# Daniel-Starr/pointcloudhookup

Measured on AMD Instinct MI355X. Metric: Mpts/s ground-filter+tower-cluster, 100 M-pt corridor; % HBM roofline on kNN, higher is better.
Workload: dtype f32 (filter) + f64 (distance predicate)

## Files before the change

### pointcloudhookup_amd/csrc/pch_filter.hip

```cpp
#include "pch_prims.h"
#include "pch_mean.h"
#include "pch_lookback.h"

namespace pch {

constexpr int SEL_BINS = 4096;
constexpr int SEL_REP0 = 4;
constexpr int SEL_TILE = 4096;

struct SelState {
    unsigned long long rank;
    unsigned long long less;
    uint32_t prefix;
    uint32_t need_next;
    uint32_t v0key;
    uint32_t pad;
};

__device__ __forceinline__ uint32_t sel_key(float v) {
    return (v != v) ? 0xFFFFFFFFu : f32_ordered(v);
}

template <int ROUNDS>
__device__ __forceinline__ void sel_hist_add(uint32_t* h, bool active, uint32_t bin) {
    bool pending = active;
#pragma unroll
    for (int round = 0; round < ROUNDS; ++round) {
        const unsigned long long todo = __ballot(pending);
        if (__popcll(todo) < 8) break;
        const int leader = (int)__builtin_ctzll(todo);
        const uint32_t b0 = (uint32_t)__builtin_amdgcn_readlane((int)bin, leader);
        const unsigned long long same = __ballot(pending && bin == b0);
        if (lane_id() == leader) atomicAdd(&h[b0], (uint32_t)__popcll(same));
        pending = pending && bin != b0;
    }
    if (pending) atomicAdd(&h[bin], 1u);
}

struct SelGate { const uint32_t* ok; const float* alt_base; const uint32_t* alt_n; };
__device__ __forceinline__ void sel_gate(const SelGate& g, const float*& base, int64_t& n, int64_t& stride) {
    if (g.ok && *g.ok) { base = g.alt_base; n = (int64_t)*g.alt_n; stride = 1; }
}

__device__ __forceinline__ float sel_key_to_float(uint32_t k) {
// ... 267 lines not shown
            float4 q[4];
#pragma unroll
            for (int r = 0; r < 4; ++r) q[r] = b4[r * 256 + threadIdx.x];
#pragma unroll
            for (int r = 0; r < 4; ++r) { take(true, q[r].x); take(true, q[r].y); take(true, q[r].z); take(true, q[r].w); }
        } else {
            for (int r = 0; r < SEL_TILE / 256; ++r) {
                const int64_t i = t0 + r * 256 + threadIdx.x;
                const bool in = i < n;
                take(in, in ? base[i] : 0.0f);
            }
        }
    }
    __syncthreads();
    flush();
    less = wave_reduce_add(less);
    nans = wave_reduce_add(nans);
    if (lane_id() == 0) {
        if (less) atomicAdd(&br->less, less);
        if (nans) atomicAdd(&br->nan, nans);
    }
}

__global__ void sel_bracket_fix_k(BrState* __restrict__ br, SelRun* __restrict__ run, unsigned long long k0, int same) {
    if (threadIdx.x != 0 || blockIdx.x != 0) return;
    const unsigned long long less = br->less, cnt = br->count;
    const bool ok = br->overflow == 0 && less <= k0 && (k0 - less) < cnt && (same || (k0 + 1 - less) < cnt);
    br->ok = ok ? 1u : 0u;
    SelState z;
    z.rank = ok ? k0 - less : k0;
    z.less = 0; z.prefix = 0; z.need_next = 0; z.v0key = 0; z.pad = 0;
    run->st[0] = z;
    run->nan_count = ok ? br->nan : 0ull;
}

__global__ __launch_bounds__(256) void sel_init_k(uint32_t* __restrict__ hist, int nwords, SelRun* __restrict__ runs,
                                                   int nruns, unsigned long long r0, unsigned long long r1,
                                                   unsigned long long r2, BrState* __restrict__ br,
                                                   uint32_t* __restrict__ also_zero, int64_t also_words) {
    const int i = blockIdx.x * 256 + threadIdx.x;
    if (i < nwords) hist[i] = 0;
    for (int64_t j = i; j < also_words; j += (int64_t)gridDim.x * 256) also_zero[j] = 0u;
    if (i < nruns) {
        SelRun z;
        memset(&z, 0, sizeof(z));
        z.st[0].rank = i == 0 ? r0 : (i == 1 ? r1 : r2);
        z.next_min = 0xFFFFFFFFu;
        runs[i] = z;
    }
    if (i == 0 && br) { BrState b; memset(&b, 0, sizeof(b)); *br = b; }
}

struct SelWs {
    float*    scal;
    SelRun*   run;
    uint32_t* hist;
    BrState*  br;
    float    *sample, *cand;
    int64_t   ns;
    uint32_t  cap;
    uint32_t* also_zero;
    int64_t   also_words;
};
static void sel_plan(Arena& a, SelWs& w, int64_t n = 0) {
    w.scal = a.take<float>(4);
    w.run = a.take<SelRun>(3);
    w.hist = a.take<uint32_t>(9 * SEL_BINS);
    w.br = nullptr; w.sample = w.cand = nullptr; w.ns = 0; w.cap = 0;
    w.also_zero = nullptr; w.also_words = 0;
    if (n >= SEL_BRACKET_MIN) {
        w.br = a.take<BrState>(1);
        w.ns = SEL_GROUP * (n / SEL_EVERY);
        w.sample = a.take<float>(w.ns);
        w.cap = (uint32_t)(n / 16) + 1024u;
        w.cand = a.take<float>(w.cap);
    }
}

struct PctIndex { int64_t k0; int same; float gamma; };
static PctIndex pct_index(int64_t n, double q_percent) {
    PctIndex r;
    const float q = (float)q_percent / 100.0f;
    const float vi = (float)(n - 1) * q;
    float prev = floorf(vi);
    r.gamma = vi - prev;
    r.same = 0;
    if (vi >= (float)(n - 1)) { prev = (float)(n - 1); r.same = 1; }
    if (vi < 0.0f) { prev = 0.0f; r.same = 1; }
    int64_t k0 = (int64_t)prev;
    if (k0 > n - 1) k0 = n - 1;
    if (k0 < 0) k0 = 0;
    if (k0 == n - 1) r.same = 1;
    r.k0 = k0;
    return r;
}

static int select_rounds(const float* base, int64_t n, int64_t stride, bool with_next, SelRun* run, uint32_t* hist,
                         hipStream_t s, SelGate gate, int64_t grid_n) {
    int64_t gb = ceil_div(grid_n, SEL_TILE);
    if (gb > 2048) gb = 2048;
    if (gb < 1) gb = 1;
    const dim3 grid((unsigned)gb), blk(256);
    PCH_LAUNCH("sel_hist0", (sel_hist_k<0, 1>), grid, blk, 0, s, base, n, stride, run, hist, gate);
    PCH_LAUNCH("sel_hist1", (sel_hist_k<1, 1>), grid, blk, 0, s, base, n, stride, run, hist, gate);
    PCH_LAUNCH("sel_hist2", (sel_hist_k<2, 1>), grid, blk, 0, s, base, n, stride, run, hist, gate);
    if (with_next) PCH_LAUNCH("sel_next", sel_next_k<>, grid, blk, 0, s, base, n, stride, run, hist, gate);
    return PCH_OK;
}

static bool select_is_bracketed(const SelWs& w, int64_t n, int64_t stride) {
    return w.sample && stride == 1 && n >= SEL_BRACKET_MIN;
}
struct SelBracket { int64_t r_lo, r_hi; };
static SelBracket select_bracket_ranks(const SelWs& w, int64_t n, const PctIndex& pi) {
    const int64_t ns = w.ns;
    const double p = (double)pi.k0 / (double)(n > 1 ? n - 1 : 1);
    const double sigma = sqrt(p * (1.0 - p) * (double)ns * 16.0);
    const int64_t margin = (int64_t)(6.0 * sigma) + ns / 500 + 16;
    const int64_t mid = (int64_t)(p * (double)(ns - 1));
    SelBracket r;
    r.r_lo = mid - margin < 0 ? 0 : mid - margin;
    r.r_hi = mid + margin > ns - 1 ? ns - 1 : mid + margin;
    return r;
}
static int select_sample_passes(const float* src, int64_t src_stride, int64_t n, double q_percent, SelWs& w,
                                hipStream_t s) {
    const PctIndex pi = pct_index(n, q_percent);
    const SelGate always = {nullptr, nullptr, nullptr};
    const SelBracket br = select_bracket_ranks(w, n, pi);
    const int64_t ns = w.ns;
    PCH_LAUNCH("sel_init", sel_init_k, dim3((unsigned)ceil_div(9 * SEL_BINS, 256)), dim3(256), 0, s, w.hist,
               9 * SEL_BINS, w.run, 3, (unsigned long long)br.r_lo, (unsigned long long)br.r_hi, 0ull, w.br,
               w.also_zero, w.also_words);
    PCH_LAUNCH("sel_sample", sel_sample_k, dim3((unsigned)ceil_div(ns, 1024)), dim3(256), 0, s, src, src_stride, ns,
               w.sample);
    int64_t gs = ceil_div(ns, SEL_TILE);
    if (gs > 2048) gs = 2048;
    if (gs < 1) gs = 1;
    const dim3 grid((unsigned)gs), blk(256);
    PCH_LAUNCH("sel_hist0", (sel_hist_k<0, 2>), grid, blk, 0, s, (const float*)w.sample, ns, (int64_t)1, w.run, w.hist, always);
    PCH_LAUNCH("sel_hist1", (sel_hist_k<1, 2>), grid, blk, 0, s, (const float*)w.sample, ns, (int64_t)1, w.run, w.hist, always);
    PCH_LAUNCH("sel_hist2", (sel_hist_k<2, 2>), grid, blk, 0, s, (const float*)w.sample, ns, (int64_t)1, w.run, w.hist, always);
    return PCH_OK;
}

static int select_passes(const float* base, int64_t n, int64_t stride, double q_percent, SelWs& w,
// ... 8 lines not shown
                   w.also_words);
        return select_rounds(base, n, stride, !pi.same, fin, hfin, s, always, n);
    }
    if (!sample_done) PCH_TRY(select_sample_passes(base, 1, n, q_percent, w, s));
    const SelBracket br = select_bracket_ranks(w, n, pi);
    const int64_t ns = w.ns;
    int64_t gb = ceil_div(n, SEL_TILE);
    {
        static int per_round[PCH_MAX_DEVICES] = {};
        const int slot = current_device_slot();
        if (!per_round[slot]) {
            int dev = 0, cus = 256;
            if (hipGetDevice(&dev) == hipSuccess) (void)hipDeviceGetAttribute(&cus, hipDeviceAttributeMultiprocessorCount, dev);
            per_round[slot] = cus * 5;
        }
        if (gb > per_round[slot]) gb = per_round[slot];
    }
    PCH_LAUNCH("sel_bracket", sel_bracket_k, dim3((unsigned)gb), dim3(256), 0, s, base, n, (const SelRun*)w.run, w.hist,
               br.r_lo == 0 ? 1 : 0, br.r_hi == ns - 1 ? 1 : 0, w.br, w.cand, w.cap);
    PCH_LAUNCH("sel_bracket_fix", sel_bracket_fix_k, dim3(1), dim3(64), 0, s, w.br, fin, (unsigned long long)pi.k0,
               pi.same);
    const SelGate src = {&w.br->ok, w.cand, &w.br->count};
    return select_rounds(base, n, stride, !pi.same, fin, hfin, s, src, n);
}
static int select_lerp(int64_t n, const float* sub, double q_percent, float add1, float add2, SelWs& w,
                       hipStream_t s) {
    const PctIndex pi = pct_index(n, q_percent);
    PCH_LAUNCH("sel_lerp", sel_lerp_k, dim3(1), dim3(256), 0, s, (const SelRun*)(w.run + 2),
               (const uint32_t*)(w.hist + 8 * SEL_BINS), pi.same ? 0 : 1, pi.same, pi.gamma, sub, add1, add2, w.scal);
    return PCH_OK;
}
static int select_percentile(const float* base, int64_t n, int64_t stride, const float* sub,
                             double q_percent, SelWs& w, hipStream_t s) {
    PCH_TRY(select_passes(base, n, stride, q_percent, w, s));
    return select_lerp(n, sub, q_percent, 0.0f, 0.0f, w, s);
}

struct SideStream { hipStream_t s; hipEvent_t ev_fork, ev_join, ev_start; bool ok; };
struct SideStreams {
    SideStream ss[PCH_MAX_DEVICES];
    SideStreams() { for (auto& x : ss) x = {nullptr, nullptr, nullptr, nullptr, false}; }
    ~SideStreams() {
        if (!may_release_hip_objects()) return;
        for (auto& x : ss)
            if (x.ok) {
                (void)hipEventDestroy(x.ev_fork); (void)hipEventDestroy(x.ev_join);
// ... 315 lines not shown
        out_scalars[5] = use_b ? 1.0f : 0.0f;
        out_scalars[6] = __uint_as_float(st->total[0]);
        out_scalars[7] = 0.0f;
        *out_count = st->failed ? (int64_t)-1 : (int64_t)st->total[use_b];
    }
    if (threadIdx.x < 6 && out_aabb) {
        const int a = threadIdx.x;
        uint32_t v = 0;
        for (int k = 0; k < GF_SLOTS; ++k) { const uint32_t u = st->slots[use_b][k][a]; v = u > v ? u : v; }
        out_aabb[a] = v == 0u ? 0.0f : f32_unordered(a < 3 ? ~v : v);
    }
}

struct GfWs {
    float*    centroid;
    float*    zcol;
    MsWs      ms;
    SelWs     sel;
    GfState*  st;
    uint64_t* status;
    size_t    clear_bytes;
    MsCand    cand;
};
static void gf_plan(Arena& a, int64_t n, GfWs& w) {
    const int64_t nb = ceil_div(n > 0 ? n : 1, GF_TILE);
    w.centroid = a.take<float>(4);
    ms_plan(a, n, w.ms);
    w.zcol = a.take<float>(n > 0 ? n : 1);
    sel_plan(a, w.sel, n);
    const size_t st_off = a.off;
    w.st = a.take<GfState>(1);
    w.status = a.take<uint64_t>(2 * nb);
    w.clear_bytes = a.off - st_off;
    const int64_t nblk = ceil_div(n > 0 ? n : 1, GF_CBLK);
    w.cand.tcand = a.take<float>(4);
    w.cand.counts = a.take<uint32_t>(nblk);
    w.cand.zsample = a.take<float>(nblk);
    w.cand.slots = a.take<float>(nblk * 4 * MS_CAND_SLOT);
    w.cand.pct = 0.0;
    w.cand.add = 0.0f;
}

}

using namespace pch;

extern "C" size_t pch_percentile_f32_ws_bytes(int64_t n) {
    Arena a;
    SelWs w;
    sel_plan(a, w, n);
    return a.off;
}

extern "C" int pch_percentile_f32(const float* base, int64_t n, int64_t stride, const float* sub,
                                  double q_percent, float* out, void* ws, size_t ws_bytes,
                                  void* stream) {
    PCH_DEVICE_GUARD(base);
    hipStream_t s = (hipStream_t)stream;
    PCH_REQUIRE(n >= 1, "percentile of an empty array (numpy raises IndexError)");
    PCH_REQUIRE(base && out && ws && stride >= 1, "bad argument");
    PCH_REQUIRE(q_percent >= 0.0 && q_percent <= 100.0, "Percentiles must be in the range [0, 100]");
    Arena a(ws, ws_bytes);
    SelWs w;
// ... 125 lines not shown
    return pch::ground_filter_run(raw, n, pct, offset, fallback_offset, min_keep, out_points, out_index, out_scalars,
                                  out_count, out_aabb, ws, ws_bytes, (hipStream_t)stream, nullptr);
}

int pch::ground_filter_run(const float* raw, int64_t n, double pct, float offset, float fallback_offset,
                           int64_t min_keep, float* out_points, int32_t* out_index, float* out_scalars,
                           int64_t* out_count, float* out_aabb, void* ws, size_t ws_bytes, hipStream_t s,
                           const GfEarly* early) {
    PCH_REQUIRE(n >= 1 && n < (int64_t(1) << 31), "n out of range [1, 2^31) (numpy raises on empty input)");
    PCH_REQUIRE(raw && out_points && out_scalars && out_count && ws, "null buffer");
    PCH_REQUIRE(pct >= 0.0 && pct <= 100.0, "Percentiles must be in the range [0, 100]");
    Arena a(ws, ws_bytes);
    GfWs w;
    gf_plan(a, n, w);
    if (a.overflow) { set_error("workspace too small: need %zu bytes", a.off); return PCH_ERR_WORKSPACE; }
    const int64_t nb = ceil_div(n, GF_TILE);

    w.cand.pct = pct;
    w.cand.add = (offset < fallback_offset ? offset : fallback_offset) - 0.5f;
    bool cand_made = false;
    w.sel.also_zero = reinterpret_cast<uint32_t*>(w.st);
    w.sel.also_words = (int64_t)(w.clear_bytes / 4);
    SideStream& ss = side_stream();
    const bool sample_early = ss.ok && select_is_bracketed(w.sel, n, 1);
    if (sample_early) {
        PCH_HIP_TRY(hipEventRecord(ss.ev_start, s));
        PCH_HIP_TRY(hipStreamWaitEvent(ss.s, ss.ev_start, 0));
        PCH_TRY(select_sample_passes(raw + 2, 3, n, pct, w.sel, ss.s));
    }
    PCH_TRY(mean_seq_launch(raw, n, w.centroid, w.ms, w.zcol, s, ss.ok ? ss.ev_fork : nullptr, nullptr, MS_DIVIDE_BY_N,
                            MS_PHASE_BOTH, &w.cand, &cand_made));
    if (ss.ok) PCH_HIP_TRY(hipStreamWaitEvent(ss.s, ss.ev_fork, 0));
    PCH_TRY(select_passes(w.zcol, n, 1, pct, w.sel, ss.ok ? ss.s : s, sample_early));
    if (ss.ok) {
        PCH_HIP_TRY(hipEventRecord(ss.ev_join, ss.s));
        PCH_HIP_TRY(hipStreamWaitEvent(s, ss.ev_join, 0));
    }
    PCH_TRY(select_lerp(n, w.centroid + 2, pct, offset, fallback_offset, w.sel, s));
    const dim3 grid((unsigned)nb), blk(GF_THREADS);
    const float* tcand = cand_made ? (const float*)w.cand.tcand : (const float*)nullptr;
    const int64_t nblk = ceil_div(n, GF_CBLK);
    const dim3 cgrid((unsigned)ceil_div(nblk, GF_CT_BLKS));
    if (cand_made)
        PCH_LAUNCH("gf_cand", gf_cand_k<0>, cgrid, blk, 0, s, (const float*)w.cand.slots, (const uint32_t*)w.cand.counts,
                   tcand, nblk, (const float*)w.centroid, (const float*)w.sel.scal, w.st, w.status, (long long)min_keep,
                   out_points, out_index);
    PCH_LAUNCH("gf_compact", gf_compact_k<0>, grid, blk, 0, s, raw, (const float*)w.zcol, n,
               (const float*)w.centroid, (const float*)w.sel.scal, w.st, w.status, (long long)min_keep, out_points,
               out_index, tcand);
    if (early) {
        PCH_LAUNCH("gf_finalize", gf_finalize_k, dim3(1), dim3(64), 0, s, (const GfState*)w.st,
                   (const float*)w.centroid, (const float*)w.sel.scal, out_scalars, out_count, out_aabb);
        PCH_TRY(peek_enqueue(early->dev, early->bytes, s));
    }
    if (cand_made)
        PCH_LAUNCH("gf_cand_fb", gf_cand_k<1>, cgrid, blk, 0, s, (const float*)w.cand.slots,
                   (const uint32_t*)w.cand.counts, tcand, nblk, (const float*)w.centroid, (const float*)w.sel.scal, w.st,
                   w.status + nb, (long long)min_keep, out_points, out_index);
    PCH_LAUNCH("gf_compact_fb", gf_compact_k<1>, grid, blk, 0, s, raw, (const float*)w.zcol, n,
               (const float*)w.centroid, (const float*)w.sel.scal, w.st, w.status + nb, (long long)min_keep, out_points,
               out_index, tcand);
    PCH_LAUNCH("gf_finalize", gf_finalize_k, dim3(1), dim3(64), 0, s, (const GfState*)w.st,
               (const float*)w.centroid, (const float*)w.sel.scal, out_scalars, out_count, out_aabb);
    return PCH_OK;
}
```

### pointcloudhookup_amd/csrc/pch_mean.h

```cpp
#pragma once
#include "pch_common.h"

namespace pch {

struct MsHdr;
struct MsRec;
struct MsPred;
constexpr int MS_CAND_SLOT = 512;
struct MsCand {
    float*    slots;
    uint32_t* counts;
    float*    tcand;
    float*    zsample;
    double    pct;
    float     add;
};
struct MsWs {
    MsPred*    pred;
    int*       stats;
    MsRec*     rec;
    MsHdr*     hdr2;
    long long* rows2;
};
void ms_plan(Arena& a, int64_t n, MsWs& w);
constexpr int64_t MS_DIVIDE_BY_N = -1, MS_NO_DIVIDE = -2;
constexpr int MS_PHASE_BOTH = 0, MS_PHASE_TABLES = 1, MS_PHASE_WALK = 2;
int mean_seq_launch(const float* xyz, int64_t n, float* out, MsWs& w, float* zcol, hipStream_t s,
                    hipEvent_t ev_zcol = nullptr, const float* sum_in = nullptr, int64_t divide_n = MS_DIVIDE_BY_N,
                    int phase = MS_PHASE_BOTH, const MsCand* cand = nullptr, bool* cand_made = nullptr);

}
```

### pointcloudhookup_amd/csrc/pch_mean.hip

```cpp
#include "pch_mean.h"

namespace pch {

constexpr int MSB       = 1024;
constexpr int MS_PER    = 16;
constexpr int MS_CAND   = 24;
constexpr int MS_ROW2   = 3 * MS_CAND;
constexpr int MS_WAVES  = 4;
constexpr uint32_t MS_NONFINITE = 1u, MS_ALLZERO = 2u;
constexpr uint32_t MS_TIGHT = 4u;
constexpr int MS_FIX_FROM = 11;
constexpr int MS_FIX_LOW  = 6;
constexpr int MS_FIX_MAX  = 16;

struct MsHdr { int emax; uint32_t tie; uint32_t flags; uint32_t mask; };
constexpr uint32_t MS_ALLCAND = (1u << MS_CAND) - 1u;
constexpr int MS_WIN = 4;

struct alignas(128) MsRec {
    MsHdr     h;
    long long A0;
    long long S[MS_CAND];
    uint32_t  fix[MS_CAND];
    uint32_t  pad[18];
// ... 56 lines not shown
        if (zsample) zsample[blk] = q.z;
    }
    const int64_t first = row * 64 * MSB;
    const double cnt_row = (double)((n - first) < (int64_t)64 * MSB ? (n - first) : (int64_t)64 * MSB);
    const double ns = (double)__popcll(__ballot(have != 0));
#pragma unroll
    for (int c = 0; c < 3; ++c) {
        const bool fin = fabs(v[c]) < 1.0e300;
        av[c] = fin ? fabs(v[c]) : 0.0;
        v[c] = fin ? v[c] : 0.0;
        double sv = v[c], sa = av[c];
#pragma unroll
        for (int o = 32; o > 0; o >>= 1) { sv += __shfl_xor(sv, o, 64); sa += __shfl_xor(sa, o, 64); }
        if (l == 0) {
            MsPred o;
            o.pre = 0.0;
            o.rowsum = ns > 0.0 ? sv / ns * cnt_row : 0.0;
            o.meanabs = ns > 0.0 ? sa / ns : 0.0;
            pred[(int64_t)c * nb2 + row] = o;
        }
    }
}

__device__ void ms_zestimate(const float* __restrict__ zs, int64_t ns, double pct, float add, float* __restrict__ tcand) {
    __shared__ uint32_t hist[2048];
    __shared__ uint32_t wsum[16];
    __shared__ uint32_t pick_bin, pick_below, total_sh;
    const int l = lane_id(), w = wave_id();
    auto add_bin = [&](bool in, uint32_t bin) {
        const unsigned long long act = __ballot(in);
        if (!act) return;
        const int lead = (int)__builtin_ctzll(act);
        const uint32_t b0 = (uint32_t)__builtin_amdgcn_readlane((int)bin, lead);
        const unsigned long long same = __ballot(in && bin == b0);
        if (l == lead) atomicAdd(&hist[b0], (uint32_t)__popcll(same));
        if (in && bin != b0) atomicAdd(&hist[bin], 1u);
    };
    auto scan_pick = [&](uint32_t rank) {
        __syncthreads();
        const uint32_t h0 = hist[2 * threadIdx.x], h1 = hist[2 * threadIdx.x + 1];
        const uint32_t incl = wave_scan_incl(h0 + h1);
        if (l == 63) wsum[w] = incl;
        __syncthreads();
        uint32_t before = incl - (h0 + h1);
        for (int k = 0; k < w; ++k) before += wsum[k];
        if (rank >= before && rank < before + h0) { pick_bin = 2 * threadIdx.x; pick_below = before; }
        else if (rank >= before + h0 && rank < before + h0 + h1) { pick_bin = 2 * threadIdx.x + 1; pick_below = before + h0; }
        __syncthreads();
    };
    for (int j = threadIdx.x; j < 2048; j += 1024) hist[j] = 0;
    if (threadIdx.x == 0) { total_sh = 0; pick_bin = 2047; pick_below = 0; }
    __syncthreads();
    constexpr int EST_STRIDE = 16, EST_BATCH = 8;
    const int64_t ne = (ns + EST_STRIDE - 1) / EST_STRIDE;
    auto for_samples = [&](auto&& f) {
        for (int64_t i0 = 0; i0 < ne; i0 += 1024 * EST_BATCH) {
            float zb[EST_BATCH];
#pragma unroll
            for (int u = 0; u < EST_BATCH; ++u) {
                const int64_t i = i0 + u * 1024 + threadIdx.x;
                zb[u] = i < ne ? zs[i * EST_STRIDE] : NAN;
            }
#pragma unroll
            for (int u = 0; u < EST_BATCH; ++u) f(zb[u]);
        }
    };
    uint32_t mine = 0;
    for_samples([&](float z) {
        const bool in = z == z;
        add_bin(in, f32_ordered(z) >> 21);
        mine += in ? 1u : 0u;
    });
// ... 2 lines not shown
    __syncthreads();
    const uint32_t total = total_sh;
    if (threadIdx.x == 0) reinterpret_cast<uint32_t*>(tcand)[1] = 0u;
    if (total == 0) { if (threadIdx.x == 0) *tcand = -INFINITY; return; }
    uint32_t rank = (uint32_t)((double)(total - 1) * (pct / 100.0));
    scan_pick(rank);
    const uint32_t top = pick_bin;
    rank -= pick_below;
    __syncthreads();
    for (int j = threadIdx.x; j < 2048; j += 1024) hist[j] = 0;
    if (threadIdx.x == 0) { pick_bin = 2047; pick_below = 0; }
    __syncthreads();
    for_samples([&](float z) {
        const uint32_t k = f32_ordered(z);
        add_bin(z == z && (k >> 21) == top, (k >> 10) & 2047u);
    });
    scan_pick(rank);
    if (threadIdx.x == 0) {
        const uint32_t key = (top << 21) | (pick_bin << 10);
        *tcand = f32_unordered(key) + add;
    }
}

__global__ __launch_bounds__(1024) void ms_prefix_k(MsPred* __restrict__ pred, int64_t nb2,
                                                    const float* __restrict__ sum_in, const float* __restrict__ zs,
                                                    int64_t ns, double pct, float add, float* __restrict__ tcand) {
    __shared__ double wsum[16];
    __shared__ double carry_sh;
    if (blockIdx.x == 3) { ms_zestimate(zs, ns, pct, add, tcand); return; }
    const int c = blockIdx.x;
    const int l = lane_id(), w = wave_id();
    if (threadIdx.x == 0) carry_sh = sum_in ? (double)sum_in[c] : 0.0;
    __syncthreads();
    for (int64_t r0 = 0; r0 < nb2; r0 += 1024) {
        const int64_t r = r0 + threadIdx.x;
        const double v = r < nb2 ? pred[(int64_t)c * nb2 + r].rowsum : 0.0;
        double incl = v;
#pragma unroll
        for (int o = 1; o < 64; o <<= 1) { const double t = __shfl_up(incl, o, 64); if (l >= o) incl += t; }
        if (l == 63) wsum[w] = incl;
        __syncthreads();
        double woff = 0.0, total = 0.0;
#pragma unroll
        for (int k = 0; k < 16; ++k) { const double t = wsum[k]; woff += k < w ? t : 0.0; total += t; }
        const double carry = carry_sh;
        if (r < nb2) pred[(int64_t)c * nb2 + r].pre = carry + woff + incl - v;
        __syncthreads();
        if (threadIdx.x == 0) carry_sh = carry + total;
        __syncthreads();
    }
}

__device__ __forceinline__ int ms_exp2_floor(double x) {
    return (int)((((unsigned long long)__double_as_longlong(x)) >> 52) & 0x7FFull) - 1023;
}

__global__ __launch_bounds__(64 * MS_WAVES) void ms_summary_k(const float* __restrict__ xyz, int64_t n,
                                                             int64_t nb, MsRec* __restrict__ recs,
                                                             float* __restrict__ zcol,
                                                             const MsPred* __restrict__ pred, int64_t nb2,
                                                             float* __restrict__ cslots, uint32_t* __restrict__ ccounts,
                                                             const float* __restrict__ tcand) {
    __shared__ __attribute__((aligned(16))) float lds[MS_WAVES][MSB * 3];
    __shared__ MsRec stage[MS_WAVES];
    const int64_t blk = (int64_t)blockIdx.x * MS_WAVES + wave_id();
    if (blk >= nb) return;
    const int l = lane_id();
    const int64_t p0 = blk * MSB;
    const int cnt = (int)((n - p0) < MSB ? (n - p0) : MSB);
    float* tile = lds[wave_id()];
    const float* src = xyz + 3 * p0;
    if (cnt == MSB) {
        const float4* s4 = reinterpret_cast<const float4*>(src);
        float4* t4 = reinterpret_cast<float4*>(tile);
#pragma unroll
        for (int i = 0; i < 12; ++i) t4[i * 64 + l] = s4[i * 64 + l];
    } else {
        for (int e = l; e < 3 * MSB; e += 64) tile[e] = e < 3 * cnt ? src[e] : 0.0f;
    }
    __builtin_amdgcn_wave_barrier();
    float zr[MS_PER];
    if (zcol || cslots) {
#pragma unroll
        for (int i = 0; i < MS_PER; ++i) zr[i] = tile[3 * (i * 64 + l) + 2];
    }
    if (zcol) {
#pragma unroll
        for (int i = 0; i < MS_PER; ++i) {
            const int p = i * 64 + l;
            if (p < cnt) zcol[p0 + p] = zr[i];
        }
    }
    if (cslots) {
        const float tc = *tcand;
        float zmax = -INFINITY;
#pragma unroll
        for (int i = 0; i < MS_PER; ++i) {
            const int p = i * 64 + l;
            if (p < cnt) zmax = fmaxf(zmax, zr[i]);
        }
        const bool some = __ballot(zmax > tc) != 0;
        uint32_t at = 0;
        if (some) {
            float* slot = cslots + blk * (4 * MS_CAND_SLOT);
#pragma unroll
            for (int i = 0; i < MS_PER; ++i) {
                const int p = i * 64 + l;
                const float z = zr[i];
                const bool take = p < cnt && z > tc;
                const unsigned long long m = __ballot(take);
                if (m == 0) continue;
                const uint32_t pos = at + (uint32_t)__popcll(m & lanemask_lt());
                if (take && pos < (uint32_t)MS_CAND_SLOT) {
// ... 706 lines not shown
                const float a0 = col[3 * (i + 0)], a1 = col[3 * (i + 1)], a2 = col[3 * (i + 2)],
                            a3 = col[3 * (i + 3)], a4 = col[3 * (i + 4)], a5 = col[3 * (i + 5)],
                            a6 = col[3 * (i + 6)], a7 = col[3 * (i + 7)];
                s = s + a0; s = s + a1; s = s + a2; s = s + a3;
                s = s + a4; s = s + a5; s = s + a6; s = s + a7;
            }
            for (; i < cnt; ++i) s = s + col[3 * i];
        }
        __syncthreads();
    }
    if (threadIdx.x < 3) out[threadIdx.x] = s / (float)n;
}

void ms_plan(Arena& a, int64_t n, MsWs& w) {
    const int64_t nb = ceil_div(n > 0 ? n : 1, MSB);
    const int64_t nb2 = ceil_div(nb, 64);
    w.stats = a.take<int>(32);
    w.pred = a.take<MsPred>(3 * nb2);
    w.rec = a.take<MsRec>(3 * nb);
    w.hdr2 = a.take<MsHdr>(3 * nb2);
    w.rows2 = a.take<long long>(3 * nb2 * MS_ROW2);
}

int mean_seq_launch(const float* xyz, int64_t n, float* out, MsWs& w, float* zcol, hipStream_t s,
                    hipEvent_t ev_zcol, const float* sum_in, int64_t divide_n, int phase, const MsCand* cand,
                    bool* cand_made) {
    if (cand_made) *cand_made = false;
    const int64_t nb = n > 0 ? ceil_div(n, MSB) : 0;
    const int64_t nb2 = ceil_div(nb, 64);
    if (n > 0 && phase != MS_PHASE_WALK) {
        static const bool no_predict = getenv("PCH_MEAN_NO_PREDICT") != nullptr;
        const MsPred* pred = nullptr;
        if (!no_predict && phase == MS_PHASE_BOTH && nb2 >= 2) {
            static const bool no_cand = getenv("PCH_GF_NO_CAND") != nullptr;
            const bool mk = cand && !no_cand;
            PCH_LAUNCH("mean_sample", ms_sample_k, dim3((unsigned)nb2), dim3(64), 0, s, xyz, n, nb, nb2, w.pred,
                       mk ? cand->zsample : (float*)nullptr);
            PCH_LAUNCH("mean_prefix", ms_prefix_k, dim3(mk ? 4 : 3), dim3(1024), 0, s, w.pred, nb2, sum_in,
                       mk ? (const float*)cand->zsample : (const float*)nullptr, nb, mk ? cand->pct : 0.0,
                       mk ? cand->add : 0.0f, mk ? cand->tcand : (float*)nullptr);
            pred = w.pred;
            if (mk && cand_made) *cand_made = true;
        }
        const bool emit = cand && cand_made && *cand_made;
        PCH_LAUNCH("mean_summary", ms_summary_k, dim3((unsigned)ceil_div(nb, MS_WAVES)), dim3(64 * MS_WAVES),
                   0, s, xyz, n, nb, w.rec, zcol, pred, nb2, emit ? cand->slots : (float*)nullptr,
                   emit ? cand->counts : (uint32_t*)nullptr, emit ? (const float*)cand->tcand : (const float*)nullptr);
        if (ev_zcol) PCH_HIP_TRY(hipEventRecord(ev_zcol, s));
        PCH_LAUNCH("mean_level2", ms_level2_k, dim3((unsigned)(3 * nb2)), dim3(256), 0, s,
                   (const MsRec*)w.rec, nb, nb2, w.hdr2, w.rows2);
    }
    if (phase == MS_PHASE_TABLES) return PCH_OK;
    MsTables T;
    T.rec = w.rec; T.nb = nb;
    T.hdr2 = w.hdr2; T.rows2 = w.rows2; T.nb2 = nb2;
    const int divide = divide_n != MS_NO_DIVIDE;
    PCH_LAUNCH("mean_walk", ms_walk_k, dim3(3), dim3(64 * MS_XW), 0, s, xyz, n, T, sum_in,
               divide_n == MS_DIVIDE_BY_N ? n : divide_n, divide, out, w.stats);
    return PCH_OK;
}

}

using namespace pch;

extern "C" size_t pch_mean_seq_f32_ws_bytes(int64_t n) {
    if (n < 0) return 0;
    Arena a;
    MsWs w;
    ms_plan(a, n, w);
// ... 38 lines not shown
```

### pointcloudhookup_amd/utils/tower_extraction.py

```python
from __future__ import annotations

import os
import sys
import time
from pathlib import Path

import numpy as np

OBB_EXTENT_ORDER = os.environ.get("PCH_OBB_EXTENT_ORDER", "unsorted")
DEVICE = os.environ.get("PCH_DEVICE", "cuda:0")
CHUNK_FAILURE = os.environ.get("PCH_CHUNK_FAILURE", "reference")
OBB_MODE = os.environ.get("PCH_OBB_MODE", "exact")
GROUND_MODE = os.environ.get("PCH_GROUND_MODE", "percentile")
GROUND_TILE = float(os.environ.get("PCH_GROUND_TILE", "20.0"))
PRESTART_BYTES = 100 << 20
CHUNK_SIZE = 50000


def extract_towers(
        input_las_path,
        progress_callback=None,
        log_callback=None,
        eps=8.0,
        min_points=80,
# ... 18 lines not shown

def _extract(input_las_path, resident_entry, progress_callback, log_callback, eps, min_points,
             aspect_ratio_threshold, min_height, max_width, min_width, duplicate_threshold):
    tower_obbs = []
    tower_rows = []

    def log(msg):
        (log_callback or print)(msg)

    def progress(value):
        if progress_callback:
            progress_callback(value)

    output_dir = Path("output_towers")
    output_dir.mkdir(exist_ok=True)

    try:
        log("📂 读取点云文件...")
        progress(5)
        import torch
        from .. import las as _las
        from .. import ops, pipeline, stages
        clock = stages.Clock("extract_towers")
        if os.path.getsize(input_las_path) >= PRESTART_BYTES:
            from .. import obb as _obb
            _obb.prestart()
        dev = torch.device(DEVICE)
        if resident_entry is not None and resident_entry.records is not None:
            hdr, XYZ = resident_entry.header, resident_entry.records
            clock.mark("LAS records taken from the device (no file read)")
        else:
            hdr, XYZ = _las.read_device(input_las_path, dev)
            clock.mark("read LAS -> device int32 (file, H2D, decode)")
        raw = ops.cast_f32(ops.las_scale(XYZ, hdr.scales, hdr.offsets))
        del XYZ
        clock.mark("int32 -> float64 -> float32")
        header_info = {"scales": hdr.scales, "offsets": hdr.offsets,
                       "point_format": hdr.point_format, "version": hdr.version}
        log(f"✅ 点云读取完成，总点数: {raw.shape[0]}")
    except Exception as e:
        log(f"⚠️ 文件读取失败: {str(e)}")
        return tower_obbs

    try:
        log("🔍 执行高度过滤...")
        progress(10)
        if raw.shape[0] == 0:
# ... 190 lines not shown
```

Baseline: 72260.

## Bracket ground percentile inside mean summary pass instead of separate sample/select passes

Extra blocks in the mean prefix kernel find low/high key brackets from a strided subsample of per-block z values. The summary kernel then counts keys below the bracket per block and writes only in-bracket z values to compacted segments, instead of writing the full z column. A collect kernel gathers those candidates into one buffer, and radix selection runs on that small set, so the separate sample passes and the full z-column write and re-read are gone. The change also enlarges the candidate buffers and, in the Python driver, measures input size from resident records rather than the file when deciding whether to prestart.

```diff
diff --git a/pointcloudhookup_amd/csrc/pch_filter.hip b/pointcloudhookup_amd/csrc/pch_filter.hip
--- a/pointcloudhookup_amd/csrc/pch_filter.hip
+++ b/pointcloudhookup_amd/csrc/pch_filter.hip
@@ -17,9 +17,6 @@
     uint32_t pad;
 };
 
-__device__ __forceinline__ uint32_t sel_key(float v) {
-    return (v != v) ? 0xFFFFFFFFu : f32_ordered(v);
-}
 
 template <int ROUNDS>
 __device__ __forceinline__ void sel_hist_add(uint32_t* h, bool active, uint32_t bin) {
@@ -333,6 +330,53 @@
     }
 }
 
+constexpr int SEL_CBLKS = 256;
+__global__ __launch_bounds__(SEL_CBLKS) void sel_collect_k(const MsBracket* __restrict__ brk,
+                                                           const MsBrRec* __restrict__ brec, int64_t nblk,
+                                                           const float* __restrict__ zseg, BrState* __restrict__ br,
+                                                           float* __restrict__ cand, uint32_t cap) {
+    __shared__ uint32_t first[SEL_CBLKS];
+    __shared__ uint32_t wtot[SEL_CBLKS / 64];
+    __shared__ uint32_t gbase;
+    if ((brk->valid[0] & brk->valid[1]) == 0u) {
+        if (blockIdx.x == 0 && threadIdx.x == 0) br->overflow = 1u;
+        return;
+    }
+    const int64_t b0 = (int64_t)blockIdx.x * SEL_CBLKS;
+    const int64_t b = b0 + threadIdx.x;
+    MsBrRec r = {0u, 0u};
+    if (b < nblk) r = brec[b];
+    const uint32_t c = r.count_less & 0xFFFFu;
+    const uint32_t incl = wave_scan_incl(c);
+    if (lane_id() == 63) wtot[wave_id()] = incl;
+    unsigned long long less = wave_reduce_add((unsigned long long)(r.count_less >> 16));
+    unsigned long long nans = wave_reduce_add((unsigned long long)r.nan);
+    if (lane_id() == 0) {
+        if (less) atomicAdd(&br->less, less);
+        if (nans) atomicAdd(&br->nan, nans);
+    }
+    __syncthreads();
+    uint32_t before = incl - c, T = 0;
+    for (int w = 0; w < SEL_CBLKS / 64; ++w) { before += w < wave_id() ? wtot[w] : 0u; T += wtot[w]; }
+    first[threadIdx.x] = before;
+    if (threadIdx.x == 0) gbase = T ? atomicAdd(&br->count, T) : 0u;
+    __syncthreads();
+    if (T == 0) return;
+    const uint32_t g0 = gbase;
+    if (g0 + T > cap || g0 + T < g0) {
+        if (threadIdx.x == 0) br->overflow = 1u;
+        return;
+    }
+#pragma unroll 4
+    for (uint32_t k = threadIdx.x; k < T; k += SEL_CBLKS) {
+        int t = 0;
+#pragma unroll
+        for (int step = SEL_CBLKS / 2; step > 0; step >>= 1)
+            if (first[t + step] <= k) t += step;
+        cand[g0 + k] = zseg[(b0 + t) * 1024 + (k - first[t])];
+    }
+}
+
 __global__ void sel_bracket_fix_k(BrState* __restrict__ br, SelRun* __restrict__ run, unsigned long long k0, int same) {
     if (threadIdx.x != 0 || blockIdx.x != 0) return;
     const unsigned long long less = br->less, cnt = br->count;
@@ -373,7 +417,7 @@
     uint32_t* also_zero;
     int64_t   also_words;
 };
-static void sel_plan(Arena& a, SelWs& w, int64_t n = 0) {
+static void sel_plan(Arena& a, SelWs& w, int64_t n = 0, bool from_summary = false) {
     w.scal = a.take<float>(4);
     w.run = a.take<SelRun>(3);
     w.hist = a.take<uint32_t>(9 * SEL_BINS);
@@ -383,7 +427,11 @@
         w.br = a.take<BrState>(1);
         w.ns = SEL_GROUP * (n / SEL_EVERY);
         w.sample = a.take<float>(w.ns);
-        w.cap = (uint32_t)(n / 16) + 1024u;
+        w.cap = (uint32_t)(n / (from_summary ? 4 : 16)) + 1024u;
+        w.cand = a.take<float>(w.cap);
+    } else if (from_summary && n > 0) {
+        w.br = a.take<BrState>(1);
+        w.cap = (uint32_t)(n / 2) + 1024u;
         w.cand = a.take<float>(w.cap);
     }
 }
@@ -423,16 +471,18 @@
     return w.sample && stride == 1 && n >= SEL_BRACKET_MIN;
 }
 struct SelBracket { int64_t r_lo, r_hi; };
-static SelBracket select_bracket_ranks(const SelWs& w, int64_t n, const PctIndex& pi) {
-    const int64_t ns = w.ns;
+static SelBracket bracket_ranks(int64_t ns, int group, int64_t n, const PctIndex& pi) {
     const double p = (double)pi.k0 / (double)(n > 1 ? n - 1 : 1);
-    const double sigma = sqrt(p * (1.0 - p) * (double)ns * 16.0);
+    const double sigma = sqrt(p * (1.0 - p) * (double)ns * (double)group);
     const int64_t margin = (int64_t)(6.0 * sigma) + ns / 500 + 16;
     const int64_t mid = (int64_t)(p * (double)(ns - 1));
     SelBracket r;
     r.r_lo = mid - margin < 0 ? 0 : mid - margin;
     r.r_hi = mid + margin > ns - 1 ? ns - 1 : mid + margin;
     return r;
+}
+static SelBracket select_bracket_ranks(const SelWs& w, int64_t n, const PctIndex& pi) {
+    return bracket_ranks(w.ns, SEL_GROUP, n, pi);
 }
 static int select_sample_passes(const float* src, int64_t src_stride, int64_t n, double q_percent, SelWs& w,
                                 hipStream_t s) {
@@ -487,6 +537,18 @@
                pi.same);
     const SelGate src = {&w.br->ok, w.cand, &w.br->count};
     return select_rounds(base, n, stride, !pi.same, fin, hfin, s, src, n);
+}
+static int select_from_summary(const float* raw, int64_t n, double q_percent, const MsCand& mc, const float* zseg,
+                               SelWs& w, hipStream_t s) {
+    const PctIndex pi = pct_index(n, q_percent);
+    SelRun* fin = w.run + 2;
+    const int64_t nblk = ceil_div(n, 1024);
+    PCH_LAUNCH("sel_collect", sel_collect_k, dim3((unsigned)ceil_div(nblk, SEL_CBLKS)), dim3(SEL_CBLKS), 0, s,
+               (const MsBracket*)mc.bracket, (const MsBrRec*)mc.brec, nblk, zseg, w.br, w.cand, w.cap);
+    PCH_LAUNCH("sel_bracket_fix", sel_bracket_fix_k, dim3(1), dim3(64), 0, s, w.br, fin, (unsigned long long)pi.k0,
+               pi.same);
+    const SelGate src = {&w.br->ok, w.cand, &w.br->count};
+    return select_rounds(raw + 2, n, 3, !pi.same, fin, w.hist + 6 * SEL_BINS, s, src, n);
 }
 static int select_lerp(int64_t n, const float* sub, double q_percent, float add1, float add2, SelWs& w,
                        hipStream_t s) {
@@ -848,12 +910,16 @@
     size_t    clear_bytes;
     MsCand    cand;
 };
+static bool gf_brackets(int64_t n) {
+    static const bool off = getenv("PCH_GF_NO_BRACKET") != nullptr;
+    return !off && ms_makes_cand(n);
+}
 static void gf_plan(Arena& a, int64_t n, GfWs& w) {
     const int64_t nb = ceil_div(n > 0 ? n : 1, GF_TILE);
     w.centroid = a.take<float>(4);
     ms_plan(a, n, w.ms);
     w.zcol = a.take<float>(n > 0 ? n : 1);
-    sel_plan(a, w.sel, n);
+    sel_plan(a, w.sel, n, gf_brackets(n));
     const size_t st_off = a.off;
     w.st = a.take<GfState>(1);
     w.status = a.take<uint64_t>(2 * nb);
@@ -865,6 +931,10 @@
     w.cand.slots = a.take<float>(nblk * 4 * MS_CAND_SLOT);
     w.cand.pct = 0.0;
     w.cand.add = 0.0f;
+    w.cand.bracket = a.take<MsBracket>(1);
+    w.cand.brec = a.take<MsBrRec>(nblk);
+    w.cand.r_lo = w.cand.r_hi = 0;
+    w.cand.force_invalid = 0;
 }
 
 }
@@ -1036,16 +1106,32 @@
     w.sel.also_zero = reinterpret_cast<uint32_t*>(w.st);
     w.sel.also_words = (int64_t)(w.clear_bytes / 4);
     SideStream& ss = side_stream();
-    const bool sample_early = ss.ok && select_is_bracketed(w.sel, n, 1);
-    if (sample_early) {
+    const bool bracket = gf_brackets(n);
+    if (bracket) {
+        static const bool invalid = getenv("PCH_GF_BRACKET_INVALID") != nullptr;
+        const int64_t nblk = ceil_div(n, GF_CBLK);
+        const SelBracket r = bracket_ranks(ceil_div(nblk, ms_bracket_stride(nblk)), 1, n, pct_index(n, pct));
+        w.cand.r_lo = r.r_lo;
+        w.cand.r_hi = r.r_hi;
+        w.cand.force_invalid = invalid ? 1 : 0;
+    } else {
+        w.cand.bracket = nullptr;
+    }
+    const bool sample_early = !bracket && ss.ok && select_is_bracketed(w.sel, n, 1);
+    if (sample_early || (bracket && ss.ok)) {
         PCH_HIP_TRY(hipEventRecord(ss.ev_start, s));
         PCH_HIP_TRY(hipStreamWaitEvent(ss.s, ss.ev_start, 0));
-        PCH_TRY(select_sample_passes(raw + 2, 3, n, pct, w.sel, ss.s));
-    }
+    }
+    if (sample_early) PCH_TRY(select_sample_passes(raw + 2, 3, n, pct, w.sel, ss.s));
+    if (bracket)
+        PCH_LAUNCH("sel_init", sel_init_k, dim3((unsigned)ceil_div(9 * SEL_BINS, 256)), dim3(256), 0, ss.ok ? ss.s : s,
+                   w.sel.hist, 9 * SEL_BINS, w.sel.run, 3, 0ull, 0ull, 0ull, w.sel.br, w.sel.also_zero, w.sel.also_words);
     PCH_TRY(mean_seq_launch(raw, n, w.centroid, w.ms, w.zcol, s, ss.ok ? ss.ev_fork : nullptr, nullptr, MS_DIVIDE_BY_N,
                             MS_PHASE_BOTH, &w.cand, &cand_made));
+    PCH_REQUIRE(!bracket || cand_made, "bracket route without candidate slots");
     if (ss.ok) PCH_HIP_TRY(hipStreamWaitEvent(ss.s, ss.ev_fork, 0));
-    PCH_TRY(select_passes(w.zcol, n, 1, pct, w.sel, ss.ok ? ss.s : s, sample_early));
+    if (bracket) PCH_TRY(select_from_summary(raw, n, pct, w.cand, w.zcol, w.sel, ss.ok ? ss.s : s));
+    else PCH_TRY(select_passes(w.zcol, n, 1, pct, w.sel, ss.ok ? ss.s : s, sample_early));
     if (ss.ok) {
         PCH_HIP_TRY(hipEventRecord(ss.ev_join, ss.s));
         PCH_HIP_TRY(hipStreamWaitEvent(s, ss.ev_join, 0));
@@ -1053,13 +1139,14 @@
     PCH_TRY(select_lerp(n, w.centroid + 2, pct, offset, fallback_offset, w.sel, s));
     const dim3 grid((unsigned)nb), blk(GF_THREADS);
     const float* tcand = cand_made ? (const float*)w.cand.tcand : (const float*)nullptr;
+    const float* zcol = bracket ? (const float*)nullptr : (const float*)w.zcol;
     const int64_t nblk = ceil_div(n, GF_CBLK);
     const dim3 cgrid((unsigned)ceil_div(nblk, GF_CT_BLKS));
     if (cand_made)
         PCH_LAUNCH("gf_cand", gf_cand_k<0>, cgrid, blk, 0, s, (const float*)w.cand.slots, (const uint32_t*)w.cand.counts,
                    tcand, nblk, (const float*)w.centroid, (const float*)w.sel.scal, w.st, w.status, (long long)min_keep,
                    out_points, out_index);
-    PCH_LAUNCH("gf_compact", gf_compact_k<0>, grid, blk, 0, s, raw, (const float*)w.zcol, n,
+    PCH_LAUNCH("gf_compact", gf_compact_k<0>, grid, blk, 0, s, raw, zcol, n,
                (const float*)w.centroid, (const float*)w.sel.scal, w.st, w.status, (long long)min_keep, out_points,
                out_index, tcand);
     if (early) {
@@ -1071,7 +1158,7 @@
         PCH_LAUNCH("gf_cand_fb", gf_cand_k<1>, cgrid, blk, 0, s, (const float*)w.cand.slots,
                    (const uint32_t*)w.cand.counts, tcand, nblk, (const float*)w.centroid, (const float*)w.sel.scal, w.st,
                    w.status + nb, (long long)min_keep, out_points, out_index);
-    PCH_LAUNCH("gf_compact_fb", gf_compact_k<1>, grid, blk, 0, s, raw, (const float*)w.zcol, n,
+    PCH_LAUNCH("gf_compact_fb", gf_compact_k<1>, grid, blk, 0, s, raw, zcol, n,
                (const float*)w.centroid, (const float*)w.sel.scal, w.st, w.status + nb, (long long)min_keep, out_points,
                out_index, tcand);
     PCH_LAUNCH("gf_finalize", gf_finalize_k, dim3(1), dim3(64), 0, s, (const GfState*)w.st,
diff --git a/pointcloudhookup_amd/csrc/pch_mean.h b/pointcloudhookup_amd/csrc/pch_mean.h
--- a/pointcloudhookup_amd/csrc/pch_mean.h
+++ b/pointcloudhookup_amd/csrc/pch_mean.h
@@ -7,6 +7,21 @@
 struct MsRec;
 struct MsPred;
 constexpr int MS_CAND_SLOT = 512;
+struct MsBracket {
+    uint32_t L, H;
+    uint32_t lo_is_min, hi_is_max;
+    uint32_t valid[2];
+    uint32_t pad[2];
+};
+struct MsBrRec { uint32_t count_less, nan; };
+constexpr int MS_BR_PER = 16;
+__host__ __device__ inline int64_t ms_bracket_stride(int64_t ns) {
+    const int64_t s = (ns + 1024 * MS_BR_PER - 1) / (1024 * MS_BR_PER);
+    return s < 1 ? 1 : s;
+}
+__device__ __forceinline__ uint32_t sel_key(float v) {
+    return (v != v) ? 0xFFFFFFFFu : f32_ordered(v);
+}
 struct MsCand {
     float*    slots;
     uint32_t* counts;
@@ -14,6 +29,10 @@
     float*    zsample;
     double    pct;
     float     add;
+    MsBracket* bracket;
+    MsBrRec*   brec;
+    int64_t    r_lo, r_hi;
+    int        force_invalid;
 };
 struct MsWs {
     MsPred*    pred;
@@ -25,6 +44,7 @@
 void ms_plan(Arena& a, int64_t n, MsWs& w);
 constexpr int64_t MS_DIVIDE_BY_N = -1, MS_NO_DIVIDE = -2;
 constexpr int MS_PHASE_BOTH = 0, MS_PHASE_TABLES = 1, MS_PHASE_WALK = 2;
+bool ms_makes_cand(int64_t n);
 int mean_seq_launch(const float* xyz, int64_t n, float* out, MsWs& w, float* zcol, hipStream_t s,
                     hipEvent_t ev_zcol = nullptr, const float* sum_in = nullptr, int64_t divide_n = MS_DIVIDE_BY_N,
                     int phase = MS_PHASE_BOTH, const MsCand* cand = nullptr, bool* cand_made = nullptr);
diff --git a/pointcloudhookup_amd/csrc/pch_mean.hip b/pointcloudhookup_amd/csrc/pch_mean.hip
--- a/pointcloudhookup_amd/csrc/pch_mean.hip
+++ b/pointcloudhookup_amd/csrc/pch_mean.hip
@@ -102,32 +102,37 @@
     }
 }
 
-__device__ void ms_zestimate(const float* __restrict__ zs, int64_t ns, double pct, float add, float* __restrict__ tcand) {
-    __shared__ uint32_t hist[2048];
-    __shared__ uint32_t wsum[16];
-    __shared__ uint32_t pick_bin, pick_below, total_sh;
+struct MsPick { uint32_t hist[2048]; uint32_t wsum[16]; uint32_t bin, below, total; };
+__device__ __forceinline__ void ms_pick_add(MsPick* P, bool in, uint32_t bin) {
+    const unsigned long long act = __ballot(in);
+    if (!act) return;
+    const int lead = (int)__builtin_ctzll(act);
+    const uint32_t b0 = (uint32_t)__builtin_amdgcn_readlane((int)bin, lead);
+    const unsigned long long same = __ballot(in && bin == b0);
+    if (lane_id() == lead) atomicAdd(&P->hist[b0], (uint32_t)__popcll(same));
+    if (in && bin != b0) atomicAdd(&P->hist[bin], 1u);
+}
+__device__ __forceinline__ void ms_pick_scan(MsPick* P, uint32_t rank) {
     const int l = lane_id(), w = wave_id();
-    auto add_bin = [&](bool in, uint32_t bin) {
-        const unsigned long long act = __ballot(in);
-        if (!act) return;
-        const int lead = (int)__builtin_ctzll(act);
-        const uint32_t b0 = (uint32_t)__builtin_amdgcn_readlane((int)bin, lead);
-        const unsigned long long same = __ballot(in && bin == b0);
-        if (l == lead) atomicAdd(&hist[b0], (uint32_t)__popcll(same));
-        if (in && bin != b0) atomicAdd(&hist[bin], 1u);
-    };
-    auto scan_pick = [&](uint32_t rank) {
-        __syncthreads();
-        const uint32_t h0 = hist[2 * threadIdx.x], h1 = hist[2 * threadIdx.x + 1];
-        const uint32_t incl = wave_scan_incl(h0 + h1);
-        if (l == 63) wsum[w] = incl;
-        __syncthreads();
-        uint32_t before = incl - (h0 + h1);
-        for (int k = 0; k < w; ++k) before += wsum[k];
-        if (rank >= before && rank < before + h0) { pick_bin = 2 * threadIdx.x; pick_below = before; }
-        else if (rank >= before + h0 && rank < before + h0 + h1) { pick_bin = 2 * threadIdx.x + 1; pick_below = before + h0; }
-        __syncthreads();
-    };
+    __syncthreads();
+    const uint32_t h0 = P->hist[2 * threadIdx.x], h1 = P->hist[2 * threadIdx.x + 1];
+    const uint32_t incl = wave_scan_incl(h0 + h1);
+    if (l == 63) P->wsum[w] = incl;
+    __syncthreads();
+    uint32_t before = incl - (h0 + h1);
+    for (int k = 0; k < w; ++k) before += P->wsum[k];
+    if (rank >= before && rank < before + h0) { P->bin = 2 * threadIdx.x; P->below = before; }
+    else if (rank >= before + h0 && rank < before + h0 + h1) { P->bin = 2 * threadIdx.x + 1; P->below = before + h0; }
+    __syncthreads();
+}
+
+__device__ void ms_zestimate(const float* __restrict__ zs, int64_t ns, double pct, float add, float* __restrict__ tcand,
+                             MsPick* P) {
+    uint32_t* hist = P->hist;
+    uint32_t &pick_bin = P->bin, &pick_below = P->below, &total_sh = P->total;
+    const int l = lane_id();
+    auto add_bin = [&](bool in, uint32_t bin) { ms_pick_add(P, in, bin); };
+    auto scan_pick = [&](uint32_t rank) { ms_pick_scan(P, rank); };
     for (int j = threadIdx.x; j < 2048; j += 1024) hist[j] = 0;
     if (threadIdx.x == 0) { total_sh = 0; pick_bin = 2047; pick_below = 0; }
     __syncthreads();
@@ -176,12 +181,55 @@
     }
 }
 
+struct MsBrArgs { MsBracket* out; int64_t stride; uint32_t rank[2]; int open[2]; int force_invalid; };
+__device__ void ms_zbracket(const float* __restrict__ zs, int64_t ns, const MsBrArgs& A, int end, MsPick* P) {
+    const int64_t ne = (ns + A.stride - 1) / A.stride;
+    uint32_t k[MS_BR_PER];
+    bool anynan = false;
+#pragma unroll
+    for (int u = 0; u < MS_BR_PER; ++u) {
+        const int64_t i = (int64_t)u * 1024 + threadIdx.x;
+        const float z = i < ne ? zs[i * A.stride] : 0.0f;
+        anynan |= z != z;
+        k[u] = f32_ordered(z);
+    }
+    if (threadIdx.x == 0) P->total = 0u;
+    uint32_t rank = A.rank[end], prefix = 0;
+#pragma unroll 1
+    for (int pass = 0; pass < 3; ++pass) {
+        const int shift = pass == 0 ? 21 : (pass == 1 ? 10 : 0), up = pass == 0 ? 32 : (pass == 1 ? 21 : 10);
+        const uint32_t bins = pass == 2 ? 1023u : 2047u;
+        __syncthreads();
+        for (int j = threadIdx.x; j < 2048; j += 1024) P->hist[j] = 0;
+        if (threadIdx.x == 0) { P->bin = bins; P->below = 0; }
+        __syncthreads();
+#pragma unroll
+        for (int u = 0; u < MS_BR_PER; ++u) {
+            const bool in = (int64_t)u * 1024 + threadIdx.x < ne && (pass == 0 || (k[u] >> up) == prefix);
+            ms_pick_add(P, in, (k[u] >> shift) & bins);
+        }
+        if (pass == 0 && __ballot(anynan) && lane_id() == 0) atomicOr(&P->total, 1u);
+        ms_pick_scan(P, rank);
+        prefix = (prefix << (pass == 2 ? 10 : 11)) | P->bin;
+        rank -= P->below;
+    }
+    if (threadIdx.x == 0) {
+        const bool valid = ne > 0 && P->total == 0u && !A.force_invalid;
+        if (end == 0) { A.out->L = A.open[0] ? 0u : prefix; A.out->lo_is_min = (uint32_t)A.open[0]; }
+        else { A.out->H = A.open[1] ? 0xFFFFFFFFu : prefix; A.out->hi_is_max = (uint32_t)A.open[1]; }
+        A.out->valid[end] = valid ? 1u : 0u;
+    }
+}
+
 __global__ __launch_bounds__(1024) void ms_prefix_k(MsPred* __restrict__ pred, int64_t nb2,
                                                     const float* __restrict__ sum_in, const float* __restrict__ zs,
-                                                    int64_t ns, double pct, float add, float* __restrict__ tcand) {
+                                                    int64_t ns, double pct, float add, float* __restrict__ tcand,
+                                                    MsBrArgs br) {
     __shared__ double wsum[16];
     __shared__ double carry_sh;
-    if (blockIdx.x == 3) { ms_zestimate(zs, ns, pct, add, tcand); return; }
+    __shared__ MsPick pick;
+    if (blockIdx.x == 3) { ms_zestimate(zs, ns, pct, add, tcand, &pick); return; }
+    if (blockIdx.x >= 4) { ms_zbracket(zs, ns, br, (int)blockIdx.x - 4, &pick); return; }
     const int c = blockIdx.x;
     const int l = lane_id(), w = wave_id();
     if (threadIdx.x == 0) carry_sh = sum_in ? (double)sum_in[c] : 0.0;
@@ -214,7 +262,9 @@
                                                              float* __restrict__ zcol,
                                                              const MsPred* __restrict__ pred, int64_t nb2,
                                                              float* __restrict__ cslots, uint32_t* __restrict__ ccounts,
-                                                             const float* __restrict__ tcand) {
+                                                             const float* __restrict__ tcand,
+                                                             const MsBracket* __restrict__ brk,
+                                                             MsBrRec* __restrict__ brec, float* __restrict__ zseg) {
     __shared__ __attribute__((aligned(16))) float lds[MS_WAVES][MSB * 3];
     __shared__ MsRec stage[MS_WAVES];
     const int64_t blk = (int64_t)blockIdx.x * MS_WAVES + wave_id();
@@ -234,7 +284,7 @@
     }
     __builtin_amdgcn_wave_barrier();
     float zr[MS_PER];
-    if (zcol || cslots) {
+    if (zcol || cslots || brk) {
 #pragma unroll
         for (int i = 0; i < MS_PER; ++i) zr[i] = tile[3 * (i * 64 + l) + 2];
     }
@@ -243,6 +293,38 @@
         for (int i = 0; i < MS_PER; ++i) {
             const int p = i * 64 + l;
             if (p < cnt) zcol[p0 + p] = zr[i];
+        }
+    }
+    if (brk) {
+        const bool valid = (brk->valid[0] & brk->valid[1]) != 0u;
+        const uint32_t L = valid ? brk->L : 1u, H = valid ? brk->H : 0u;
+        uint32_t tally = 0, mask = 0;
+#pragma unroll
+        for (int i = 0; i < MS_PER; ++i) {
+            const bool in = i * 64 + l < cnt;
+            const uint32_t k = sel_key(zr[i]);
+            tally += (in && k < L ? 1u : 0u) + (in && zr[i] != zr[i] ? 0x10000u : 0u);
+            mask |= (in && k >= L && k <= H) ? (1u << i) : 0u;
+        }
+        tally = ms_wave_all(tally, [](uint32_t a, uint32_t b) { return a + b; });
+        uint32_t total = 0;
+        if (__ballot(mask != 0u)) {
+            const uint32_t mine = (uint32_t)__popc(mask);
+            const uint32_t incl = wave_scan_incl(mine);
+            total = (uint32_t)__builtin_amdgcn_readlane((int)incl, 63);
+            float* __restrict__ seg = zseg + p0;
+            uint32_t pos = incl - mine;
+            while (mask) {
+                const int i = __ffs((int)mask) - 1;
+                mask &= mask - 1u;
+                seg[pos++] = tile[3 * (i * 64 + l) + 2];
+            }
+        }
+        if (l == 0) {
+            MsBrRec r;
+            r.count_less = total | ((tally & 0xFFFFu) << 16);
+            r.nan = tally >> 16;
+            brec[blk] = r;
         }
     }
     if (cslots) {
@@ -995,6 +1077,15 @@
     w.rows2 = a.take<long long>(3 * nb2 * MS_ROW2);
 }
 
+static bool ms_predicts(int64_t n, int phase) {
+    static const bool no_predict = getenv("PCH_MEAN_NO_PREDICT") != nullptr;
+    return !no_predict && phase == MS_PHASE_BOTH && ceil_div(ceil_div(n, MSB), 64) >= 2;
+}
+bool ms_makes_cand(int64_t n) {
+    static const bool no_cand = getenv("PCH_GF_NO_CAND") != nullptr;
+    return n > 0 && !no_cand && ms_predicts(n, MS_PHASE_BOTH);
+}
+
 int mean_seq_launch(const float* xyz, int64_t n, float* out, MsWs& w, float* zcol, hipStream_t s,
                     hipEvent_t ev_zcol, const float* sum_in, int64_t divide_n, int phase, const MsCand* cand,
                     bool* cand_made) {
@@ -1002,23 +1093,36 @@
     const int64_t nb = n > 0 ? ceil_div(n, MSB) : 0;
     const int64_t nb2 = ceil_div(nb, 64);
     if (n > 0 && phase != MS_PHASE_WALK) {
-        static const bool no_predict = getenv("PCH_MEAN_NO_PREDICT") != nullptr;
         const MsPred* pred = nullptr;
-        if (!no_predict && phase == MS_PHASE_BOTH && nb2 >= 2) {
-            static const bool no_cand = getenv("PCH_GF_NO_CAND") != nullptr;
-            const bool mk = cand && !no_cand;
+        bool bracket = false;
+        if (ms_predicts(n, phase)) {
+            const bool mk = cand && ms_makes_cand(n);
+            bracket = mk && cand->bracket;
+            MsBrArgs ba;
+            memset(&ba, 0, sizeof(ba));
+            if (bracket) {
+                ba.out = cand->bracket;
+                ba.stride = ms_bracket_stride(nb);
+                const int64_t ne = ceil_div(nb, ba.stride);
+                ba.rank[0] = (uint32_t)cand->r_lo; ba.rank[1] = (uint32_t)cand->r_hi;
+                ba.open[0] = cand->r_lo == 0; ba.open[1] = cand->r_hi == ne - 1;
+                ba.force_invalid = cand->force_invalid;
+            }
             PCH_LAUNCH("mean_sample", ms_sample_k, dim3((unsigned)nb2), dim3(64), 0, s, xyz, n, nb, nb2, w.pred,
                        mk ? cand->zsample : (float*)nullptr);
-            PCH_LAUNCH("mean_prefix", ms_prefix_k, dim3(mk ? 4 : 3), dim3(1024), 0, s, w.pred, nb2, sum_in,
+            PCH_LAUNCH("mean_prefix", ms_prefix_k, dim3(mk ? (bracket ? 6 : 4) : 3), dim3(1024), 0, s, w.pred, nb2, sum_in,
                        mk ? (const float*)cand->zsample : (const float*)nullptr, nb, mk ? cand->pct : 0.0,
-                       mk ? cand->add : 0.0f, mk ? cand->tcand : (float*)nullptr);
+                       mk ? cand->add : 0.0f, mk ? cand->tcand : (float*)nullptr, ba);
             pred = w.pred;
             if (mk && cand_made) *cand_made = true;
         }
         const bool emit = cand && cand_made && *cand_made;
         PCH_LAUNCH("mean_summary", ms_summary_k, dim3((unsigned)ceil_div(nb, MS_WAVES)), dim3(64 * MS_WAVES),
-                   0, s, xyz, n, nb, w.rec, zcol, pred, nb2, emit ? cand->slots : (float*)nullptr,
-                   emit ? cand->counts : (uint32_t*)nullptr, emit ? (const float*)cand->tcand : (const float*)nullptr);
+                   0, s, xyz, n, nb, w.rec, bracket ? (float*)nullptr : zcol, pred, nb2,
+                   emit ? cand->slots : (float*)nullptr, emit ? cand->counts : (uint32_t*)nullptr,
+                   emit ? (const float*)cand->tcand : (const float*)nullptr,
+                   bracket ? (const MsBracket*)cand->bracket : (const MsBracket*)nullptr,
+                   bracket ? cand->brec : (MsBrRec*)nullptr, bracket ? zcol : (float*)nullptr);
         if (ev_zcol) PCH_HIP_TRY(hipEventRecord(ev_zcol, s));
         PCH_LAUNCH("mean_level2", ms_level2_k, dim3((unsigned)(3 * nb2)), dim3(256), 0, s,
                    (const MsRec*)w.rec, nb, nb2, w.hdr2, w.rows2);
diff --git a/pointcloudhookup_amd/utils/tower_extraction.py b/pointcloudhookup_amd/utils/tower_extraction.py
--- a/pointcloudhookup_amd/utils/tower_extraction.py
+++ b/pointcloudhookup_amd/utils/tower_extraction.py
@@ -64,7 +64,11 @@
         from .. import las as _las
         from .. import ops, pipeline, stages
         clock = stages.Clock("extract_towers")
-        if os.path.getsize(input_las_path) >= PRESTART_BYTES:
+        if resident_entry is not None and resident_entry.records is not None:
+            in_bytes = int(resident_entry.records.shape[0]) * _las.RECORD_LEN[resident_entry.header.point_format]
+        else:
+            in_bytes = os.path.getsize(input_las_path)
+        if in_bytes >= PRESTART_BYTES:
             from .. import obb as _obb
             _obb.prestart()
         dev = torch.device(DEVICE)
```

Result: faster. 73470 (median of 6 runs) (+1.7%).
